# imatge-upc/rsis

Measured on AMD Instinct MI355X. Metric: training images/sec at 256x256, T=10, batch=32 per GPU, higher is better.
Workload: dtype f32

## Files before the change

rsis_amd/csrc/conv_wgrad_tiled.hip:

```cpp
#include "common.h"
#include "launchers.h"
#include "limb_split.h"
#include "wgrad_block_order.h"
#include "wgrad_parts.h"
#include <stdlib.h>
#include <string.h>

typedef __bf16 wg_bf16x8 __attribute__((ext_vector_type(8)));
typedef unsigned wg_u32x4 __attribute__((ext_vector_type(4)));

#define WG_LIMB_PRODUCTS 6
[[maybe_unused]] __device__ constexpr int wg_limb_pa[9] = {2, 1, 0, 1, 0, 0, 2, 1, 2};
[[maybe_unused]] __device__ constexpr int wg_limb_pb[9] = {0, 1, 2, 0, 1, 0, 1, 2, 2};

__device__ __forceinline__ void wg_limb_pack8(const float (&v)[8], wg_bf16x8 (&out)[3]) {
  wg_u32x4 q[3];
#pragma unroll
  for (int m = 0; m < 4; ++m) {
    float lo[3], hi[3];
    rsis_limb_split3(v[2 * m], lo[0], lo[1], lo[2]);
    rsis_limb_split3(v[2 * m + 1], hi[0], hi[1], hi[2]);
    q[0][m] = __builtin_amdgcn_perm(__float_as_uint(v[2 * m + 1]), __float_as_uint(v[2 * m]), 0x07060302u);
    q[1][m] = __builtin_amdgcn_perm(__float_as_uint(hi[1]), __float_as_uint(lo[1]), 0x07060302u);
    q[2][m] = __builtin_amdgcn_perm(__float_as_uint(hi[2]), __float_as_uint(lo[2]), 0x07060302u);
  }
#pragma unroll
  for (int l = 0; l < 3; ++l) out[l] = __builtin_bit_cast(wg_bf16x8, q[l]);
}

struct WgradTiledArgs {
  const float* dy;
  const float* x;
  float* dw;
  int B, Cs, H, W, Cout;
  int ldo, n_off, interleave_hid;
  int n_co_tiles, n_n_tiles, n_sp_tiles, tiles_per_split;
};

template <int BM, int BN, int WGM, int WGN, int KS, int TW, int KSP = 1, int RAG = 0, int LIMB = 0>
__device__ __forceinline__ void wgrad_tiled_body(const WgradTiledArgs& p, const int bx, const int by) {
#if __HIP_DEVICE_COMPILE__
  constexpr int TM = BM / WGM / 32, TN = BN / WGN / 32;
  constexpr int KK = KS * KS, HALO = KS / 2;
  constexpr int TP = KS == 1 ? 32 : 64;
  constexpr int TH = TP / TW;
  constexpr int NG = TP / 4;
  constexpr int GPR = TW / 4;
  constexpr int PW = TW + 2 * HALO, PH = TH + 2 * HALO, IMS = PW * PH;
  constexpr int CI_P = KS == 1 ? BN : (BN + KK - 2) / KK + 1;
  constexpr int AS = BM * TP;
  constexpr int XS = KS == 1 ? BN * TP : (CI_P * IMS + 255) / 256 * 256;
  constexpr int NA = BM * NG / 256;
  constexpr int NB4 = KS == 1 ? BN * NG / 256 : 0;
  constexpr int NB1 = KS == 1 ? 0 : XS / 256;
  static_assert(WGM * WGN * KSP == 4 && (BM * NG) % 256 == 0 && (KS == 3 || (BN * NG) % 256 == 0) && (NG / 2) % KSP == 0 && (NG / 2 / KSP) % 2 == 0, "config");

  __shared__ __attribute__((aligned(16))) float lds[2 * (AS + XS)];
  float* const As0 = lds;
  float* const Xs0 = lds + 2 * AS;

  const int tid = threadIdx.x, lane = tid & 63, l31 = lane & 31, hi = lane >> 5;
  const int wave = __builtin_amdgcn_readfirstlane(tid >> 6);
  const int wk = wave / (WGM * WGN), wm = (wave % (WGM * WGN)) / WGN, wn = wave % WGN;
  const int H = p.H, W = p.W, HW = H * W, Cs = p.Cs, Cout = p.Cout;
  const int co_t = bx % p.n_co_tiles, n_t = bx / p.n_co_tiles;
  const int co0 = co_t * BM, n0 = n_t * BN;
  const int ci0 = n0 / KK;
  const int Nn = Cs * KK;
  const int tiles_x = RAG ? (W + TW - 1) / TW : W / TW, tiles_y = RAG ? (H + TH - 1) / TH : H / TH;
  const int rx = W - (tiles_x - 1) * TW, ry = H - (tiles_y - 1) * TH;
  const int t_begin = by * p.tiles_per_split;
  const int t_end = min(t_begin + p.tiles_per_split, p.n_sp_tiles);
  if (t_begin >= t_end) return;

  unsigned voa[NA];
#pragma unroll
  for (int i = 0; i < NA; ++i) {
    const int idx = tid + i * 256;
    const int row = idx / NG, sl = idx % NG;
    const int G = (sl & ~7) | ((sl & 7) ^ (row & 7));
    const int y = G / GPR, x4 = G % GPR;
    voa[i] = co0 + row < Cout ? ((unsigned)((co0 + row) * HW + y * W + x4 * 4) * 4u) | (RAG == 2 && x4 * 4 >= rx ? 1u : 0u) | (RAG == 2 && y >= ry ? 2u : 0u) : RSIS_OOB;
  }
  unsigned voa1[RAG == 1 ? 4 * NA : 1];
  unsigned vob1r[RAG == 1 && NB4 ? 4 * NB4 : 1];
  if constexpr (RAG == 1) {
#pragma unroll
    for (int k = 0; k < 4 * NA; ++k) {
      const int P = k * 256 + tid, idx = P >> 2, e = P & 3;
      const int row = idx / NG, sl = idx % NG;
      const int G = (sl & ~7) | ((sl & 7) ^ (row & 7));
      const int y = G / GPR, x = (G % GPR) * 4 + e;
      voa1[k] = co0 + row < Cout ? ((unsigned)((co0 + row) * HW + y * W + x) * 4u) | (x >= rx ? 1u : 0u) | (y >= ry ? 2u : 0u) : RSIS_OOB;
    }
    if constexpr (KS == 1) {
#pragma unroll
      for (int k = 0; k < 4 * NB4; ++k) {
        const int P = k * 256 + tid, idx = P >> 2, e = P & 3;
        const int row = idx / NG, sl = idx % NG;
        const int G = (sl & ~7) | ((sl & 7) ^ (row & 7));
        const int y = G / GPR, x = (G % GPR) * 4 + e;
        vob1r[k] = n0 + row < Cs ? ((unsigned)((n0 + row) * HW + y * W + x) * 4u) | (x >= rx ? 1u : 0u) | (y >= ry ? 2u : 0u) : RSIS_OOB;
      }
    }
  }
  unsigned vob4[NB4 ? NB4 : 1];
  unsigned vob1[NB1 ? NB1 : 1];
  unsigned cls1[NB1 ? NB1 : 1];
  if constexpr (KS == 1) {
#pragma unroll
    for (int i = 0; i < NB4; ++i) {
      const int idx = tid + i * 256;
      const int row = idx / NG, sl = idx % NG;
      const int G = (sl & ~7) | ((sl & 7) ^ (row & 7));
      const int y = G / GPR, x4 = G % GPR;
      vob4[i] = n0 + row < Cs ? ((unsigned)((n0 + row) * HW + y * W + x4 * 4) * 4u) | (RAG == 2 && x4 * 4 >= rx ? 1u : 0u) | (RAG == 2 && y >= ry ? 2u : 0u) : RSIS_OOB;
    }
  } else {
#pragma unroll
    for (int i = 0; i < NB1; ++i) {
      const int e = tid + i * 256;
      const int cl = e / IMS, rem = e - cl * IMS;
      const int py = rem / PW, pxx = rem - py * PW;
      const bool ok = cl < CI_P && ci0 + cl < Cs;
      vob1[i] = ok ? (unsigned)(cl * HW + py * W + pxx) * 4u : RSIS_OOB;
      cls1[i] = (py == 0 ? 1u : 0u) | (py - 1 >= ry ? 2u : 0u) | (pxx == 0 ? 4u : 0u) | (pxx - 1 >= rx ? 8u : 0u);
    }
  }

  int sg[NG / 2 / KSP];
  int bo[NG / 2 / KSP];
#pragma unroll
  for (int gg = 0; gg < NG / 2 / KSP; ++gg) {
    const int g = gg * KSP + (KSP == 1 ? 0 : wk);
    sg[gg] = ((2 * g + hi) ^ (l31 & 7)) * 4;
    bo[gg] = KS == 1 ? 0 : (g / (TW / 8)) * PW + (g % (TW / 8)) * 8;
  }
  const int arow = (wm * TM * 32 + l31) * TP;
  int xb[TN];
#pragma unroll
  for (int j = 0; j < TN; ++j) {
    const int nl = wn * TN * 32 + j * 32 + l31;
    if constexpr (KS == 1) {
      xb[j] = nl * TP;
    } else {
      const int n = n0 + nl;
      const int cl = n / KK - ci0, rs = n - (n / KK) * KK;
      xb[j] = cl * IMS + (rs / KS) * PW + (rs % KS) + 4 * hi;
    }
  }

  f32x16 acc[TM][TN];
#pragma unroll
  for (int i = 0; i < TM; ++i)
#pragma unroll
    for (int j = 0; j < TN; ++j)
#pragma unroll
      for (int r = 0; r < 16; ++r) acc[i][j][r] = 0.f;

  int tb = t_begin / (tiles_x * tiles_y);
  int trem = t_begin - tb * (tiles_x * tiles_y);
  int ty = trem / tiles_x, tx = trem - ty * tiles_x;

#define WG_ISSUE(BUF)                                                                                          \
  {                                                                                                            \
    const int y0 = ty * TH, x0 = tx * TW;                                                                      \
    const float* ab = p.dy + ((size_t)tb * Cout * HW + y0 * W + x0);                                           \
    const __amdgpu_buffer_rsrc_t ra_ = __builtin_amdgcn_make_buffer_rsrc((void*)ab, 0, 0x7FFFFFF0, 0x00020000); \
    const unsigned lastm = (tx == tiles_x - 1 ? 1u : 0u) | (ty == tiles_y - 1 ? 2u : 0u);                      \
    if constexpr (RAG == 1) {                                                                                  \
      float* As = As0 + (BUF) * AS + wave * 64;                                                                \
      _Pragma("unroll") for (int k = 0; k < 4 * NA; ++k)                                                       \
        __builtin_amdgcn_raw_ptr_buffer_load_lds(ra_, (lds_vp_t)(As + k * 256), 4, (voa1[k] & lastm) ? RSIS_OOB : (voa1[k] & ~3u), 0, 0, 0); \
    } else {                                                                                                   \
      float* As = As0 + (BUF) * AS + wave * 256;                                                               \
      _Pragma("unroll") for (int i = 0; i < NA; ++i)                                                           \
        __builtin_amdgcn_raw_ptr_buffer_load_lds(ra_, (lds_vp_t)(As + i * 1024), 16,                           \
                                                 RAG == 2 ? ((voa[i] & lastm) ? RSIS_OOB : (voa[i] & ~3u)) : voa[i], 0, 0, 0); \
    }                                                                                                          \
    if constexpr (KS == 1) {                                                                                   \
      const float* bb = p.x + ((size_t)tb * Cs * HW + y0 * W + x0);                                            \
      const __amdgpu_buffer_rsrc_t rb_ = __builtin_amdgcn_make_buffer_rsrc((void*)bb, 0, 0x7FFFFFF0, 0x00020000); \
      if constexpr (RAG == 1) {                                                                                \
        float* Xs = Xs0 + (BUF) * XS + wave * 64;                                                              \
        _Pragma("unroll") for (int k = 0; k < 4 * NB4; ++k)                                                    \
          __builtin_amdgcn_raw_ptr_buffer_load_lds(rb_, (lds_vp_t)(Xs + k * 256), 4, (vob1r[k] & lastm) ? RSIS_OOB : (vob1r[k] & ~3u), 0, 0, 0); \
      } else {                                                                                                 \
        float* Xs = Xs0 + (BUF) * XS + wave * 256;                                                             \
        _Pragma("unroll") for (int i = 0; i < NB4; ++i)                                                        \
          __builtin_amdgcn_raw_ptr_buffer_load_lds(rb_, (lds_vp_t)(Xs + i * 1024), 16,                         \
                                                   RAG == 2 ? ((vob4[i] & lastm) ? RSIS_OOB : (vob4[i] & ~3u)) : vob4[i], 0, 0, 0); \
      }                                                                                                        \
    } else {                                                                                                   \
      const float* bb = p.x + (((size_t)tb * Cs + ci0) * HW + (y0 - 1) * W + (x0 - 1));                        \
      const __amdgpu_buffer_rsrc_t rb_ = __builtin_amdgcn_make_buffer_rsrc((void*)bb, 0, 0x7FFFFFF0, 0x00020000); \
      const unsigned edge = (y0 == 0 ? 1u : 0u) | (ty == tiles_y - 1 ? 2u : 0u) | (x0 == 0 ? 4u : 0u) | (tx == tiles_x - 1 ? 8u : 0u); \
      float* Xs = Xs0 + (BUF) * XS + wave * 64;                                                                \
      _Pragma("unroll") for (int i = 0; i < NB1; ++i) {                                                        \
        const unsigned vo = (cls1[i] & edge) ? RSIS_OOB : vob1[i];                                             \
        __builtin_amdgcn_raw_ptr_buffer_load_lds(rb_, (lds_vp_t)(Xs + i * 256), 4, vo, 0, 0, 0);               \
      }                                                                                                        \
    }                                                                                                          \
    if (++tx == tiles_x) { tx = 0; if (++ty == tiles_y) { ty = 0; ++tb; } }                                    \
  }
#define WG_LAND() __builtin_amdgcn_s_waitcnt(0x0F70);

  WG_ISSUE(0)
  WG_LAND()
  __syncthreads();
  const int ntl = t_end - t_begin;
  for (int t = 0; t < ntl; ++t) {
    const int cur = t & 1;
    if (t + 1 < ntl) WG_ISSUE(cur ^ 1)
    {
      const float* As = As0 + cur * AS + arow;
      const float* Xs = Xs0 + cur * XS;
      if constexpr (LIMB) {
#pragma unroll
        for (int g = 0; g < NG / 2 / KSP; g += 2) {
          wg_bf16x8 al[TM][3], bl[TN][3];
#pragma unroll
          for (int i = 0; i < TM; ++i) {
            const f32x4 a0 = *reinterpret_cast<const f32x4*>(As + i * 32 * TP + sg[g]);
            const f32x4 a1 = *reinterpret_cast<const f32x4*>(As + i * 32 * TP + sg[g + 1]);
            const float v[8] = {a0[0], a0[1], a0[2], a0[3], a1[0], a1[1], a1[2], a1[3]};
            wg_limb_pack8(v, al[i]);
          }
#pragma unroll
          for (int j = 0; j < TN; ++j) {
            float v[8];
            if constexpr (KS == 1) {
              const f32x4 b0 = *reinterpret_cast<const f32x4*>(Xs + xb[j] + sg[g]);
              const f32x4 b1 = *reinterpret_cast<const f32x4*>(Xs + xb[j] + sg[g + 1]);
#pragma unroll
              for (int e = 0; e < 4; ++e) { v[e] = b0[e]; v[4 + e] = b1[e]; }
            } else {
#pragma unroll
              for (int u = 0; u < 2; ++u)
#pragma unroll
                for (int e = 0; e < 4; ++e)
                  v[4 * u + e] = Xs[xb[j] + (KSP == 1 ? ((g + u) / (TW / 8)) * PW + ((g + u) % (TW / 8)) * 8 : bo[g + u]) + e];
            }
            wg_limb_pack8(v, bl[j]);
          }
#pragma unroll
          for (int q = 0; q < WG_LIMB_PRODUCTS; ++q)
#pragma unroll
            for (int i = 0; i < TM; ++i)
#pragma unroll
              for (int j = 0; j < TN; ++j)
                acc[i][j] = __builtin_amdgcn_mfma_f32_32x32x16_bf16(al[i][wg_limb_pa[q]], bl[j][wg_limb_pb[q]], acc[i][j], 0, 0, 0);
        }
      } else
#pragma unroll
      for (int g = 0; g < NG / 2 / KSP; ++g) {
        f32x4 a4[TM];
#pragma unroll
        for (int i = 0; i < TM; ++i) a4[i] = *reinterpret_cast<const f32x4*>(As + i * 32 * TP + sg[g]);
        if constexpr (KS == 1) {
          f32x4 b4[TN];
#pragma unroll
          for (int j = 0; j < TN; ++j) b4[j] = *reinterpret_cast<const f32x4*>(Xs + xb[j] + sg[g]);
#pragma unroll
          for (int e = 0; e < 4; ++e)
#pragma unroll
            for (int i = 0; i < TM; ++i)
#pragma unroll
              for (int j = 0; j < TN; ++j) acc[i][j] = __builtin_amdgcn_mfma_f32_32x32x2f32(a4[i][e], b4[j][e], acc[i][j], 0, 0, 0);
        } else {
#pragma unroll
          for (int e = 0; e < 4; ++e) {
            float b[TN];
#pragma unroll
            for (int j = 0; j < TN; ++j) b[j] = Xs[xb[j] + (KSP == 1 ? (g / (TW / 8)) * PW + (g % (TW / 8)) * 8 : bo[g]) + e];
#pragma unroll
            for (int i = 0; i < TM; ++i)
#pragma unroll
              for (int j = 0; j < TN; ++j) acc[i][j] = __builtin_amdgcn_mfma_f32_32x32x2f32(a4[i][e], b[j], acc[i][j], 0, 0, 0);
          }
        }
      }
    }
    WG_LAND()
    __syncthreads();
  }
#undef WG_ISSUE
#undef WG_LAND

  wg_atomic_tiles<TM, TN>(acc, p.dw, Cout, p.ldo, p.n_off, p.interleave_hid, co0 + wm * TM * 32 + 4 * hi, n0 + wn * TN * 32 + l31, Nn);
#endif
}

#define RSIS_WG_MAXJ 48
struct WgradTiledGroup {
  int n;
  int xcd_order;
  int begin[RSIS_WG_MAXJ + 1];
  WgradTiledArgs job[RSIS_WG_MAXJ];
};
static_assert(sizeof(WgradTiledGroup) <= 4000, "kernel arguments are limited to 4 KB");

template <int BM, int BN, int WGM, int WGN, int KS, int TW, int KSP = 1, int RAG = 0, int LIMB = 0>
__global__ __launch_bounds__(256) void conv_wgrad_tiled_group_kernel(const WgradTiledGroup g) {
  const int b = g.xcd_order ? rsis_xcd_logical_block(blockIdx.x, gridDim.x) : (int)blockIdx.x;
  int lo = 0, hi = g.n - 1;
  while (lo < hi) {
    const int mid = (lo + hi + 1) >> 1;
    if (g.begin[mid] <= b) lo = mid; else hi = mid - 1;
  }
  const WgradTiledArgs& p = g.job[lo];
  const int local = b - g.begin[lo];
  const int ntile = p.n_co_tiles * p.n_n_tiles;
  wgrad_tiled_body<BM, BN, WGM, WGN, KS, TW, KSP, RAG, LIMB>(p, local % ntile, local / ntile);
}

static unsigned wg_limb_mask(int ks, int tw) {
  if (ks == 3) return tw == 16 ? 0x3Fu : (tw == 8 ? 1u << 5 : 0u);
  return (tw == 16 || tw == 8 ? 1u << 2 : 0u) | 1u << 5;
}
static bool wg_use_limbs(int ks, int tw, int code, int rag) {
  static const int mode = [] {
    const char* e = getenv("RSIS_WGRAD_LIMBS");
    if (!e || !e[0]) return 0;
    if (e[0] == '0') return 1;
    return strcmp(e, "all") == 0 ? 2 : 0;
  }();
  if (mode) return mode == 2;
  return rag == 0 && ((wg_limb_mask(ks, tw) >> code) & 1u);
}

static unsigned wg_xcd_mask(int ks, int tw) {
  if (ks == 3) return tw == 16 ? 0x5u : 0u;
  return tw == 32 ? 1u << 5 : 0u;
}
static int wg_xcd_order(int ks, int tw, int code, int rag) {
  static const int mode = [] {
    const char* e = getenv("RSIS_WGRAD_XCD");
    if (!e || !e[0]) return 0;
    if (e[0] == '0') return 1;
    return strcmp(e, "all") == 0 ? 2 : 0;
  }();
  if (mode) return mode == 2;
  return rag == 0 && ((wg_xcd_mask(ks, tw) >> code) & 1u);
}
static constexpr int tiled_code_of(int bm, int bn) { return bm == 32 ? (bn == 64 ? 0 : 1) : (bm == 64 ? (bn == 64 ? 2 : 3) : (bn == 64 ? 4 : 5)); }

static int tiled_tw(int H, int W, int ks) {
  const int tp = ks == 1 ? 32 : 64;
  for (int tw = ks == 1 ? 32 : 16; tw >= 8; tw >>= 1)
    if (W % tw == 0 && H % (tp / tw) == 0) return tw;
  return 0;
}
static int tiled_tw_ragged(int W, int ks) {
  const int wide = ks == 1 ? 32 : 16;
  return W > 16 ? wide : (W > 8 ? 16 : 8);
}

static int tiled_cfg_code_single(const WgradTiledArgs& a, int ks) {
  const int nmod = (a.Cs * ks * ks) % 128;
  const bool narrow = nmod != 0 && nmod <= 64;
  if (ks == 1 && a.Cout > 32) return 2;
  if (a.Cout <= 32) return narrow && !rsis_deterministic() ? 0 : 1;
  if (a.Cout <= 64) return narrow ? 2 : 3;
  return narrow ? 4 : 5;
}

static int wg_job_class(const WgradTiledArgs& a, int ks) {
  if (ks == 1) return a.Cout <= 32 ? -1 : (a.Cout >= 128 && a.Cs >= 128 ? 1 : 0);
  const int nmod = (a.Cs * ks * ks) % 128;
  if (nmod == 0 || nmod > 64) return -1;
  return a.Cout <= 32 ? 0 : (a.Cout <= 64 ? 1 : 2);
}
static int wg_wide_code(int ks, int cls) { return ks == 1 ? 5 : 2 * cls + 1; }
static int wg_group_tile(int ks, int tw, int cls) {
  return ks == 1 && cls == 1 && (tw == 32 || tw == 16) ? 5 : -1;
}
static int tiled_cfg_code(const WgradTiledArgs& a, int ks, int tw, bool grouped) {
  static const int mode = [] {
    const char* e = getenv("RSIS_WGRAD_TILES");
    if (!e || !e[0]) return 0;
    if (strcmp(e, "0") == 0) return 1;
    return strcmp(e, "wide") == 0 ? 2 : 0;
  }();
  const int single = tiled_cfg_code_single(a, ks);
  const int cls = wg_job_class(a, ks);
  if (!grouped || cls < 0 || mode == 1 || rsis_deterministic()) return single;
  const int code = mode == 2 ? wg_wide_code(ks, cls) : wg_group_tile(ks, tw, cls);
  return code < 0 ? single : code;
}

static void tiled_split_plan(WgradTiledArgs* jobs, int n, int ks, bool big_tile, bool alone, int rag) {
  if (alone && rag == 0) {
    WgradTiledArgs& a = jobs[0];
    const int ntile = a.n_co_tiles * a.n_n_tiles;
    const int slots = ks == 1 ? (big_tile ? 256 : 512) : 256 * (big_tile ? 2 : 3);
    int nsplit = ntile >= slots ? 1 : slots / ntile;
    if (nsplit > a.n_sp_tiles / 2) nsplit = a.n_sp_tiles / 2;
    if (nsplit < 1 || rsis_deterministic()) nsplit = 1;
    a.tiles_per_split = rsis_cdiv(a.n_sp_tiles, nsplit);
    return;
  }
  long total_iters = 0;
  for (int j = 0; j < n; ++j) total_iters += (long)jobs[j].n_co_tiles * jobs[j].n_n_tiles * jobs[j].n_sp_tiles;
  static const int env_tb = getenv("RSIS_WG_GROUP_BLOCKS") ? atoi(getenv("RSIS_WG_GROUP_BLOCKS")) : 0;
  const long target_blocks = env_tb > 0 ? env_tb : 2048;
  long L = (total_iters + target_blocks - 1) / target_blocks;
  if (L < 2) L = 2;
  if (rsis_deterministic()) L = 1L << 40;
  for (int j = 0; j < n; ++j) {
    int nsplit = rsis_cdiv(jobs[j].n_sp_tiles, L);
    if (nsplit < 1) nsplit = 1;
    jobs[j].tiles_per_split = rsis_cdiv(jobs[j].n_sp_tiles, nsplit);
  }
}

template <int BM, int BN, int WGM, int WGN, int KS, int TW, int KSP = 1, int RAG = 0, int LIMB = 0>
static int launch_group_cfg(WgradTiledArgs* jobs, int n, bool alone, hipStream_t st) {
  constexpr int TH = (KS == 1 ? 32 : 64) / TW;
  for (int j = 0; j < n; ++j) {
    WgradTiledArgs& a = jobs[j];
    a.n_co_tiles = rsis_cdiv(a.Cout, BM);
    a.n_n_tiles = rsis_cdiv((long)a.Cs * KS * KS, BN);
    a.n_sp_tiles = RAG ? a.B * rsis_cdiv(a.H, TH) * rsis_cdiv(a.W, TW) : a.B * (a.H / TH) * (a.W / TW);
  }
  tiled_split_plan(jobs, n, KS, BM * BN >= 128 * 128, alone, RAG);
  for (int j0 = 0; j0 < n; j0 += RSIS_WG_MAXJ) {
    WgradTiledGroup g;
    g.xcd_order = !alone && wg_xcd_order(KS, TW, tiled_code_of(BM, BN), RAG);
    g.n = n - j0 < RSIS_WG_MAXJ ? n - j0 : RSIS_WG_MAXJ;
    int blocks = 0;
    for (int j = 0; j < g.n; ++j) {
      const WgradTiledArgs& a = jobs[j0 + j];
      g.begin[j] = blocks;
      g.job[j] = a;
      blocks += a.n_co_tiles * a.n_n_tiles * rsis_cdiv(a.n_sp_tiles, a.tiles_per_split);
    }
    g.begin[g.n] = blocks;
    hipLaunchKernelGGL((conv_wgrad_tiled_group_kernel<BM, BN, WGM, WGN, KS, TW, KSP, RAG, LIMB>), dim3(blocks), dim3(256), 0, st, g);
    if (rsis_check_launch() != RSIS_OK) return RSIS_ERR_LAUNCH;
  }
  return RSIS_OK;
}

template <int KS, int TW, int RAG, int LIMB>
static int launch_group_code(int code, WgradTiledArgs* jobs, int n, bool alone, hipStream_t st) {
  switch (code) {
    case 0: return launch_group_cfg<32, 64, 1, 2, KS, TW, 2, RAG, LIMB>(jobs, n, alone, st);
    case 1: return launch_group_cfg<32, 128, 1, 4, KS, TW, 1, RAG, LIMB>(jobs, n, alone, st);
    case 2: return launch_group_cfg<64, 64, 2, 2, KS, TW, 1, RAG, LIMB>(jobs, n, alone, st);
    case 3: return launch_group_cfg<64, 128, 2, 2, KS, TW, 1, RAG, LIMB>(jobs, n, alone, st);
    case 4: return launch_group_cfg<128, 64, 2, 2, KS, TW, 1, RAG, LIMB>(jobs, n, alone, st);
    default: return launch_group_cfg<128, 128, 2, 2, KS, TW, 1, RAG, LIMB>(jobs, n, alone, st);
  }
}

template <int KS, int TW>
static int launch_group_tw(int rag, int code, WgradTiledArgs* jobs, int n, bool alone, hipStream_t st) {
  const bool limb = wg_use_limbs(KS, TW, code, rag);
  switch (rag * 2 + limb) {
    case 0: return launch_group_code<KS, TW, 0, 0>(code, jobs, n, alone, st);
    case 1: return launch_group_code<KS, TW, 0, 1>(code, jobs, n, alone, st);
    case 2: return launch_group_code<KS, TW, 1, 0>(code, jobs, n, alone, st);
    case 3: return launch_group_code<KS, TW, 1, 1>(code, jobs, n, alone, st);
    case 4: return launch_group_code<KS, TW, 2, 0>(code, jobs, n, alone, st);
    default: return launch_group_code<KS, TW, 2, 1>(code, jobs, n, alone, st);
  }
}

static int launch_group(int ks, int tw, int rag, int code, WgradTiledArgs* jobs, int n, bool alone, hipStream_t st) {
  if (ks == 1 && tw == 32) return launch_group_tw<1, 32>(rag, code, jobs, n, alone, st);
  if (ks == 1 && tw == 16) return launch_group_tw<1, 16>(rag, code, jobs, n, alone, st);
  if (ks == 1 && tw == 8) return launch_group_tw<1, 8>(rag, code, jobs, n, alone, st);
  if (ks == 3 && tw == 16) return launch_group_tw<3, 16>(rag, code, jobs, n, alone, st);
  if (ks == 3 && tw == 8) return launch_group_tw<3, 8>(rag, code, jobs, n, alone, st);
  return RSIS_ERR_ARG;
}

static WgradTiledArgs tiled_args(const WgradArgs& w) {
  WgradTiledArgs a = {};
  a.dy = w.dy; a.x = w.x; a.dw = w.dw; a.B = w.B; a.Cs = w.Cs; a.H = w.H; a.W = w.W; a.Cout = w.Cout;
  a.ldo = w.ldo; a.n_off = w.n_off; a.interleave_hid = w.interleave_hid;
  return a;
}

static int tiled_launch_jobs(const WgradArgs* w, int n, int ks, bool alone, hipStream_t st) {
  if (n < 1) return RSIS_OK;
  WgradTiledArgs* all = (WgradTiledArgs*)malloc(sizeof(WgradTiledArgs) * n * 2);
  int* key = (int*)malloc(sizeof(int) * n);
  if (!all || !key) { free(all); free(key); return RSIS_ERR_LAUNCH; }
  WgradTiledArgs* bucket = all + n;
  for (int j = 0; j < n; ++j) {
    WgradTiledArgs& a = all[j] = tiled_args(w[j]);
    const int twa = tiled_tw(a.H, a.W, ks);
    if (twa) key[j] = twa * 8 + tiled_cfg_code(a, ks, twa, !alone);
    else {
      if (ks == 1 && (a.H * a.W) % 4 == 0) { a.W = a.H * a.W; a.H = 1; }
      key[j] = (a.W % 4 == 0 ? 2048 : 1024) + tiled_tw_ragged(a.W, ks) * 8 + tiled_cfg_code_single(a, ks);
    }
  }
  int rc = RSIS_OK;
  for (int j = 0; j < n && rc == RSIS_OK; ++j) {
    if (key[j] < 0) continue;
    const int k = key[j];
    int m = 0;
    for (int i = j; i < n; ++i)
      if (key[i] == k) { bucket[m++] = all[i]; key[i] = -1; }
    rc = launch_group(ks, (k & 1023) / 8, k >> 10, k % 8, bucket, m, alone, st);
  }
  free(all); free(key);
  return rc;
}

int rsis_launch_conv_wgrad_tiled_group(const WgradArgs* w, int n, int ks, hipStream_t st) { return tiled_launch_jobs(w, n, ks, false, st); }
int rsis_launch_conv_wgrad_tiled(const WgradArgs& w, int ks, hipStream_t st) { return tiled_launch_jobs(&w, 1, ks, true, st); }

bool rsis_wgrad_tiled_supported(const WgradArgs& w, int ks) {
  if (!(ks == 1 || ks == 3) || w.stride != 1 || w.pad != ks / 2 || w.H != w.Ho || w.W != w.Wo) return false;
  static const bool ragged_on = !(getenv("RSIS_WGRAD_RAGGED") && getenv("RSIS_WGRAD_RAGGED")[0] == '0');
  if (tiled_tw(w.H, w.W, ks) == 0 && !ragged_on) return false;
  const long img = (long)w.H * w.W * 4;
  return (long)w.Cout * img < (1L << 30) && (long)w.Cs * img < (1L << 30);
}
```

Before: 970.2.

## Extend tiled MFMA weight-gradient kernel to stride-2 3x3 and 7x7 convolutions

Adds a stride-2 variant of the tiled weight-gradient kernel. It stages a full-resolution input patch into LDS with 16-byte buffer loads and reads it with stride-2 offsets. Stride-2 3x3 convolutions and 7x7 convolutions with few input channels now use this path instead of the previous fallback. The limb path accumulates each tile into a separate register partial before adding it to the main accumulator. This costs extra registers but should reduce rounding error.

```diff
diff --git a/rsis_amd/csrc/conv_wgrad_tiled.hip b/rsis_amd/csrc/conv_wgrad_tiled.hip
--- a/rsis_amd/csrc/conv_wgrad_tiled.hip
+++ b/rsis_amd/csrc/conv_wgrad_tiled.hip
@@ -3,6 +3,7 @@
 #include "limb_split.h"
 #include "wgrad_block_order.h"
 #include "wgrad_parts.h"
+#include "wgrad_strided_map.h"
 #include <stdlib.h>
 #include <string.h>
 
@@ -37,7 +38,7 @@
   int n_co_tiles, n_n_tiles, n_sp_tiles, tiles_per_split;
 };
 
-template <int BM, int BN, int WGM, int WGN, int KS, int TW, int KSP = 1, int RAG = 0, int LIMB = 0>
+template <int BM, int BN, int WGM, int WGN, int KS, int TW, int KSP = 1, int RAG = 0, int LIMB = 0, int STR = 1>
 __device__ __forceinline__ void wgrad_tiled_body(const WgradTiledArgs& p, const int bx, const int by) {
 #if __HIP_DEVICE_COMPILE__
   constexpr int TM = BM / WGM / 32, TN = BN / WGN / 32;
@@ -46,14 +47,17 @@
   constexpr int TH = TP / TW;
   constexpr int NG = TP / 4;
   constexpr int GPR = TW / 4;
-  constexpr int PW = TW + 2 * HALO, PH = TH + 2 * HALO, IMS = PW * PH;
+  constexpr int PW = STR == 2 ? wgs2_pitch(KS, TW) : TW + 2 * HALO;
+  constexpr int IMS = STR == 2 ? wgs2_chan(KS, TW, TH) : PW * (TH + 2 * HALO);
   constexpr int CI_P = KS == 1 ? BN : (BN + KK - 2) / KK + 1;
   constexpr int AS = BM * TP;
-  constexpr int XS = KS == 1 ? BN * TP : (CI_P * IMS + 255) / 256 * 256;
+  constexpr int XS = KS == 1 ? BN * TP : (STR == 2 ? wgs2_groups(KS, TW, TH, CI_P) * 4 : (CI_P * IMS + 255) / 256 * 256);
   constexpr int NA = BM * NG / 256;
   constexpr int NB4 = KS == 1 ? BN * NG / 256 : 0;
-  constexpr int NB1 = KS == 1 ? 0 : XS / 256;
-  static_assert(WGM * WGN * KSP == 4 && (BM * NG) % 256 == 0 && (KS == 3 || (BN * NG) % 256 == 0) && (NG / 2) % KSP == 0 && (NG / 2 / KSP) % 2 == 0, "config");
+  constexpr int NB1 = KS == 1 ? 0 : (STR == 2 ? (XS / 4 + 255) / 256 : XS / 256);
+  static_assert(WGM * WGN * KSP == 4 && (BM * NG) % 256 == 0 && (KS != 1 || (BN * NG) % 256 == 0) && (NG / 2) % KSP == 0 && (NG / 2 / KSP) % 2 == 0, "config");
+  static_assert(STR == 1 ? KS == 1 || KS == 3 : STR == 2 && (KS == 3 || KS == 7) && RAG == 0, "stride 2: 3x3 / 7x7 on maps of whole tiles");
+  static_assert(2 * (AS + XS) * 4 <= WG_CU_LDS, "LDS of a CU");
 
   __shared__ __attribute__((aligned(16))) float lds[2 * (AS + XS)];
   float* const As0 = lds;
@@ -63,6 +67,7 @@
   const int wave = __builtin_amdgcn_readfirstlane(tid >> 6);
   const int wk = wave / (WGM * WGN), wm = (wave % (WGM * WGN)) / WGN, wn = wave % WGN;
   const int H = p.H, W = p.W, HW = H * W, Cs = p.Cs, Cout = p.Cout;
+  const int Wx = STR * W, HWx = STR * STR * HW;
   const int co_t = bx % p.n_co_tiles, n_t = bx / p.n_co_tiles;
   const int co0 = co_t * BM, n0 = n_t * BN;
   const int ci0 = n0 / KK;
@@ -120,6 +125,12 @@
 #pragma unroll
     for (int i = 0; i < NB1; ++i) {
       const int e = tid + i * 256;
+      if constexpr (STR == 2) {
+        const WgS2Group s = wgs2_group(KS, TW, TH, CI_P, e);
+        vob1[i] = s.staged && ci0 + s.cl < Cs ? (unsigned)(s.cl * HWx + s.row * Wx + 4 * s.g4) * 4u : RSIS_OOB;
+        cls1[i] = wgs2_class(KS, TW, TH, s.row, s.g4);
+        continue;
+      }
       const int cl = e / IMS, rem = e - cl * IMS;
       const int py = rem / PW, pxx = rem - py * PW;
       const bool ok = cl < CI_P && ci0 + cl < Cs;
@@ -134,7 +145,7 @@
   for (int gg = 0; gg < NG / 2 / KSP; ++gg) {
     const int g = gg * KSP + (KSP == 1 ? 0 : wk);
     sg[gg] = ((2 * g + hi) ^ (l31 & 7)) * 4;
-    bo[gg] = KS == 1 ? 0 : (g / (TW / 8)) * PW + (g % (TW / 8)) * 8;
+    bo[gg] = KS == 1 ? 0 : STR * ((g / (TW / 8)) * PW + (g % (TW / 8)) * 8);
   }
   const int arow = (wm * TM * 32 + l31) * TP;
   int xb[TN];
@@ -146,7 +157,7 @@
     } else {
       const int n = n0 + nl;
       const int cl = n / KK - ci0, rs = n - (n / KK) * KK;
-      xb[j] = cl * IMS + (rs / KS) * PW + (rs % KS) + 4 * hi;
+      xb[j] = (STR == 2 ? wgs2_base(KS, TW, TH, cl, rs / KS, rs % KS) : cl * IMS + (rs / KS) * PW + (rs % KS)) + STR * 4 * hi;
     }
   }
 
@@ -192,13 +203,16 @@
                                                    RAG == 2 ? ((vob4[i] & lastm) ? RSIS_OOB : (vob4[i] & ~3u)) : vob4[i], 0, 0, 0); \
       }                                                                                                        \
     } else {                                                                                                   \
-      const float* bb = p.x + (((size_t)tb * Cs + ci0) * HW + (y0 - 1) * W + (x0 - 1));                        \
+      const float* bb = p.x + (((size_t)tb * Cs + ci0) * HWx + (STR * y0 - HALO) * Wx + (STR * x0 - (STR == 2 ? WGS2_LEFT : HALO))); \
       const __amdgpu_buffer_rsrc_t rb_ = __builtin_amdgcn_make_buffer_rsrc((void*)bb, 0, 0x7FFFFFF0, 0x00020000); \
       const unsigned edge = (y0 == 0 ? 1u : 0u) | (ty == tiles_y - 1 ? 2u : 0u) | (x0 == 0 ? 4u : 0u) | (tx == tiles_x - 1 ? 8u : 0u); \
-      float* Xs = Xs0 + (BUF) * XS + wave * 64;                                                                \
+      float* Xs = Xs0 + (BUF) * XS + wave * (STR == 2 ? 256 : 64);                                             \
       _Pragma("unroll") for (int i = 0; i < NB1; ++i) {                                                        \
         const unsigned vo = (cls1[i] & edge) ? RSIS_OOB : vob1[i];                                             \
-        __builtin_amdgcn_raw_ptr_buffer_load_lds(rb_, (lds_vp_t)(Xs + i * 256), 4, vo, 0, 0, 0);               \
+        if constexpr (STR == 2) {                                                                              \
+          if (i * 256 + wave * 64 < XS / 4)            \
+            __builtin_amdgcn_raw_ptr_buffer_load_lds(rb_, (lds_vp_t)(Xs + i * 1024), 16, vo, 0, 0, 0);         \
+        } else __builtin_amdgcn_raw_ptr_buffer_load_lds(rb_, (lds_vp_t)(Xs + i * 256), 4, vo, 0, 0, 0);        \
       }                                                                                                        \
     }                                                                                                          \
     if (++tx == tiles_x) { tx = 0; if (++ty == tiles_y) { ty = 0; ++tb; } }                                    \
@@ -216,6 +230,16 @@
       const float* As = As0 + cur * AS + arow;
       const float* Xs = Xs0 + cur * XS;
       if constexpr (LIMB) {
+        constexpr bool FLUSH = STR == 2;
+        f32x16 part[TM][TN];
+        if constexpr (FLUSH) {
+#pragma unroll
+          for (int i = 0; i < TM; ++i)
+#pragma unroll
+            for (int j = 0; j < TN; ++j)
+#pragma unroll
+              for (int r = 0; r < 16; ++r) part[i][j][r] = 0.f;
+        }
 #pragma unroll
         for (int g = 0; g < NG / 2 / KSP; g += 2) {
           wg_bf16x8 al[TM][3], bl[TN][3];
@@ -239,7 +263,7 @@
               for (int u = 0; u < 2; ++u)
 #pragma unroll
                 for (int e = 0; e < 4; ++e)
-                  v[4 * u + e] = Xs[xb[j] + (KSP == 1 ? ((g + u) / (TW / 8)) * PW + ((g + u) % (TW / 8)) * 8 : bo[g + u]) + e];
+                  v[4 * u + e] = Xs[xb[j] + (KSP == 1 ? STR * (((g + u) / (TW / 8)) * PW + ((g + u) % (TW / 8)) * 8) : bo[g + u]) + STR * e];
             }
             wg_limb_pack8(v, bl[j]);
           }
@@ -249,7 +273,14 @@
             for (int i = 0; i < TM; ++i)
 #pragma unroll
               for (int j = 0; j < TN; ++j)
-                acc[i][j] = __builtin_amdgcn_mfma_f32_32x32x16_bf16(al[i][wg_limb_pa[q]], bl[j][wg_limb_pb[q]], acc[i][j], 0, 0, 0);
+                if constexpr (FLUSH) part[i][j] = __builtin_amdgcn_mfma_f32_32x32x16_bf16(al[i][wg_limb_pa[q]], bl[j][wg_limb_pb[q]], part[i][j], 0, 0, 0);
+                else acc[i][j] = __builtin_amdgcn_mfma_f32_32x32x16_bf16(al[i][wg_limb_pa[q]], bl[j][wg_limb_pb[q]], acc[i][j], 0, 0, 0);
+        }
+        if constexpr (FLUSH) {
+#pragma unroll
+          for (int i = 0; i < TM; ++i)
+#pragma unroll
+            for (int j = 0; j < TN; ++j) acc[i][j] += part[i][j];
         }
       } else
 #pragma unroll
@@ -272,7 +303,7 @@
           for (int e = 0; e < 4; ++e) {
             float b[TN];
 #pragma unroll
-            for (int j = 0; j < TN; ++j) b[j] = Xs[xb[j] + (KSP == 1 ? (g / (TW / 8)) * PW + (g % (TW / 8)) * 8 : bo[g]) + e];
+            for (int j = 0; j < TN; ++j) b[j] = Xs[xb[j] + (KSP == 1 ? STR * ((g / (TW / 8)) * PW + (g % (TW / 8)) * 8) : bo[g]) + STR * e];
 #pragma unroll
             for (int i = 0; i < TM; ++i)
 #pragma unroll
@@ -300,7 +331,7 @@
 };
 static_assert(sizeof(WgradTiledGroup) <= 4000, "kernel arguments are limited to 4 KB");
 
-template <int BM, int BN, int WGM, int WGN, int KS, int TW, int KSP = 1, int RAG = 0, int LIMB = 0>
+template <int BM, int BN, int WGM, int WGN, int KS, int TW, int KSP = 1, int RAG = 0, int LIMB = 0, int STR = 1>
 __global__ __launch_bounds__(256) void conv_wgrad_tiled_group_kernel(const WgradTiledGroup g) {
   const int b = g.xcd_order ? rsis_xcd_logical_block(blockIdx.x, gridDim.x) : (int)blockIdx.x;
   int lo = 0, hi = g.n - 1;
@@ -311,14 +342,30 @@
   const WgradTiledArgs& p = g.job[lo];
   const int local = b - g.begin[lo];
   const int ntile = p.n_co_tiles * p.n_n_tiles;
-  wgrad_tiled_body<BM, BN, WGM, WGN, KS, TW, KSP, RAG, LIMB>(p, local % ntile, local / ntile);
+  wgrad_tiled_body<BM, BN, WGM, WGN, KS, TW, KSP, RAG, LIMB, STR>(p, local % ntile, local / ntile);
 }
 
 static unsigned wg_limb_mask(int ks, int tw) {
   if (ks == 3) return tw == 16 ? 0x3Fu : (tw == 8 ? 1u << 5 : 0u);
   return (tw == 16 || tw == 8 ? 1u << 2 : 0u) | 1u << 5;
 }
-static bool wg_use_limbs(int ks, int tw, int code, int rag) {
+static int wg_s2_class(int ks) { return ks == 7 ? 1 : 0; }
+static unsigned wg_s2_class_mask() { return 0x3u; }
+static unsigned wg_s2_limb_mask() { return 0x1u; }
+static bool wg_s2_on(int ks) {
+  static const int mode = [] {
+    const char* e = getenv("RSIS_WGRAD_S2");
+    if (!e || !e[0]) return -1;
+    if (strcmp(e, "0") == 0) return 0;
+    if (strcmp(e, "3") == 0) return 1;
+    if (strcmp(e, "7") == 0) return 2;
+    return strcmp(e, "all") == 0 ? 3 : -1;
+  }();
+  return ((mode < 0 ? wg_s2_class_mask() : (unsigned)mode) >> wg_s2_class(ks)) & 1u;
+}
+static int wg_s2_code(int ks) { return ks == 7 ? 2 : 3; }
+
+static bool wg_use_limbs(int ks, int tw, int code, int rag, int str = 1) {
   static const int mode = [] {
     const char* e = getenv("RSIS_WGRAD_LIMBS");
     if (!e || !e[0]) return 0;
@@ -326,6 +373,7 @@
     return strcmp(e, "all") == 0 ? 2 : 0;
   }();
   if (mode) return mode == 2;
+  if (str == 2) return (wg_s2_limb_mask() >> wg_s2_class(ks)) & 1u;
   return rag == 0 && ((wg_limb_mask(ks, tw) >> code) & 1u);
 }
 
@@ -333,7 +381,7 @@
   if (ks == 3) return tw == 16 ? 0x5u : 0u;
   return tw == 32 ? 1u << 5 : 0u;
 }
-static int wg_xcd_order(int ks, int tw, int code, int rag) {
+static int wg_xcd_order(int ks, int tw, int code, int rag, int str = 1) {
   static const int mode = [] {
     const char* e = getenv("RSIS_WGRAD_XCD");
     if (!e || !e[0]) return 0;
@@ -341,6 +389,7 @@
     return strcmp(e, "all") == 0 ? 2 : 0;
   }();
   if (mode) return mode == 2;
+  if (str == 2) return 0;
   return rag == 0 && ((wg_xcd_mask(ks, tw) >> code) & 1u);
 }
 static constexpr int tiled_code_of(int bm, int bn) { return bm == 32 ? (bn == 64 ? 0 : 1) : (bm == 64 ? (bn == 64 ? 2 : 3) : (bn == 64 ? 4 : 5)); }
@@ -414,7 +463,7 @@
   }
 }
 
-template <int BM, int BN, int WGM, int WGN, int KS, int TW, int KSP = 1, int RAG = 0, int LIMB = 0>
+template <int BM, int BN, int WGM, int WGN, int KS, int TW, int KSP = 1, int RAG = 0, int LIMB = 0, int STR = 1>
 static int launch_group_cfg(WgradTiledArgs* jobs, int n, bool alone, hipStream_t st) {
   constexpr int TH = (KS == 1 ? 32 : 64) / TW;
   for (int j = 0; j < n; ++j) {
@@ -426,7 +475,7 @@
   tiled_split_plan(jobs, n, KS, BM * BN >= 128 * 128, alone, RAG);
   for (int j0 = 0; j0 < n; j0 += RSIS_WG_MAXJ) {
     WgradTiledGroup g;
-    g.xcd_order = !alone && wg_xcd_order(KS, TW, tiled_code_of(BM, BN), RAG);
+    g.xcd_order = !alone && wg_xcd_order(KS, TW, tiled_code_of(BM, BN), RAG, STR);
     g.n = n - j0 < RSIS_WG_MAXJ ? n - j0 : RSIS_WG_MAXJ;
     int blocks = 0;
     for (int j = 0; j < g.n; ++j) {
@@ -436,7 +485,7 @@
       blocks += a.n_co_tiles * a.n_n_tiles * rsis_cdiv(a.n_sp_tiles, a.tiles_per_split);
     }
     g.begin[g.n] = blocks;
-    hipLaunchKernelGGL((conv_wgrad_tiled_group_kernel<BM, BN, WGM, WGN, KS, TW, KSP, RAG, LIMB>), dim3(blocks), dim3(256), 0, st, g);
+    hipLaunchKernelGGL((conv_wgrad_tiled_group_kernel<BM, BN, WGM, WGN, KS, TW, KSP, RAG, LIMB, STR>), dim3(blocks), dim3(256), 0, st, g);
     if (rsis_check_launch() != RSIS_OK) return RSIS_ERR_LAUNCH;
   }
   return RSIS_OK;
@@ -467,7 +516,26 @@
   }
 }
 
-static int launch_group(int ks, int tw, int rag, int code, WgradTiledArgs* jobs, int n, bool alone, hipStream_t st) {
+template <int KS, int TW>
+static int launch_group_s2(int code, WgradTiledArgs* jobs, int n, bool alone, hipStream_t st) {
+  const bool limb = wg_use_limbs(KS, TW, code, 0, 2);
+  if constexpr (KS == 7) {
+    if (code != 2) return RSIS_ERR_ARG;
+    return limb ? launch_group_cfg<64, 64, 2, 2, KS, TW, 1, 0, 1, 2>(jobs, n, alone, st) : launch_group_cfg<64, 64, 2, 2, KS, TW, 1, 0, 0, 2>(jobs, n, alone, st);
+  } else {
+    if (code != 3) return RSIS_ERR_ARG;
+    return limb ? launch_group_cfg<64, 128, 2, 2, KS, TW, 1, 0, 1, 2>(jobs, n, alone, st) : launch_group_cfg<64, 128, 2, 2, KS, TW, 1, 0, 0, 2>(jobs, n, alone, st);
+  }
+}
+
+static int launch_group(int ks, int str, int tw, int rag, int code, WgradTiledArgs* jobs, int n, bool alone, hipStream_t st) {
+  if (str == 2) {
+    if (ks == 3 && tw == 16) return launch_group_s2<3, 16>(code, jobs, n, alone, st);
+    if (ks == 3 && tw == 8) return launch_group_s2<3, 8>(code, jobs, n, alone, st);
+    if (ks == 7 && tw == 16) return launch_group_s2<7, 16>(code, jobs, n, alone, st);
+    if (ks == 7 && tw == 8) return launch_group_s2<7, 8>(code, jobs, n, alone, st);
+    return RSIS_ERR_ARG;
+  }
   if (ks == 1 && tw == 32) return launch_group_tw<1, 32>(rag, code, jobs, n, alone, st);
   if (ks == 1 && tw == 16) return launch_group_tw<1, 16>(rag, code, jobs, n, alone, st);
   if (ks == 1 && tw == 8) return launch_group_tw<1, 8>(rag, code, jobs, n, alone, st);
@@ -491,6 +559,11 @@
   WgradTiledArgs* bucket = all + n;
   for (int j = 0; j < n; ++j) {
     WgradTiledArgs& a = all[j] = tiled_args(w[j]);
+    if (w[j].stride == 2) {
+      a.H = w[j].Ho; a.W = w[j].Wo;
+      key[j] = 4096 + tiled_tw(a.H, a.W, ks) * 8 + wg_s2_code(ks);
+      continue;
+    }
     const int twa = tiled_tw(a.H, a.W, ks);
     if (twa) key[j] = twa * 8 + tiled_cfg_code(a, ks, twa, !alone);
     else {
@@ -505,7 +578,7 @@
     int m = 0;
     for (int i = j; i < n; ++i)
       if (key[i] == k) { bucket[m++] = all[i]; key[i] = -1; }
-    rc = launch_group(ks, (k & 1023) / 8, k >> 10, k % 8, bucket, m, alone, st);
+    rc = launch_group(ks, k >> 12 ? 2 : 1, (k & 1023) / 8, (k >> 10) & 3, k % 8, bucket, m, alone, st);
   }
   free(all); free(key);
   return rc;
@@ -515,6 +588,13 @@
 int rsis_launch_conv_wgrad_tiled(const WgradArgs& w, int ks, hipStream_t st) { return tiled_launch_jobs(&w, 1, ks, true, st); }
 
 bool rsis_wgrad_tiled_supported(const WgradArgs& w, int ks) {
+  if (w.stride == 2) {
+    if (!((ks == 3 || (ks == 7 && w.Cs <= 4)) && w.pad == ks / 2 && wg_s2_on(ks))) return false;
+    if (w.H != 2 * w.Ho || w.W != 2 * w.Wo || tiled_tw(w.Ho, w.Wo, ks) == 0) return false;
+    if ((size_t)w.x & 15) return false;
+    const long img = (long)w.H * w.W * 4;
+    return (long)w.Cout * img < (1L << 30) && (long)w.Cs * img < (1L << 30);
+  }
   if (!(ks == 1 || ks == 3) || w.stride != 1 || w.pad != ks / 2 || w.H != w.Ho || w.W != w.Wo) return false;
   static const bool ragged_on = !(getenv("RSIS_WGRAD_RAGGED") && getenv("RSIS_WGRAD_RAGGED")[0] == '0');
   if (tiled_tw(w.H, w.W, ks) == 0 && !ragged_on) return false;
diff --git a/rsis_amd/csrc/wgrad_strided_map.h b/rsis_amd/csrc/wgrad_strided_map.h
--- /dev/null
+++ b/rsis_amd/csrc/wgrad_strided_map.h
@@ -0,0 +1,35 @@
+#pragma once
+
+#if defined(__HIPCC__) || defined(__CUDACC__)
+#define RSIS_S2MAP_HD __host__ __device__
+#else
+#define RSIS_S2MAP_HD
+#endif
+
+RSIS_S2MAP_HD constexpr int wgs2_tap_p(int ks, int r) { return (r - ks / 2) & 1; }
+RSIS_S2MAP_HD constexpr int wgs2_tap_a(int ks, int r) { return (r - ks / 2 - wgs2_tap_p(ks, r)) / 2; }
+RSIS_S2MAP_HD constexpr int wgs2_extent(int ks, int t, int p) { return t + (ks / 2 - p) / 2 + (ks / 2 + p) / 2; }
+RSIS_S2MAP_HD constexpr int wgs2_span(int ks, int t) { return wgs2_extent(ks, t, 0) + wgs2_extent(ks, t, 1); }
+
+constexpr int WGS2_LEFT = 4;
+RSIS_S2MAP_HD constexpr int wgs2_pitch(int ks, int tw) { return (WGS2_LEFT - ks / 2 + wgs2_span(ks, tw) + 3) / 4 * 4; }
+RSIS_S2MAP_HD constexpr int wgs2_chan(int ks, int tw, int th) { return wgs2_span(ks, th) * wgs2_pitch(ks, tw) + (ks == 3 ? 4 : 0); }
+RSIS_S2MAP_HD constexpr int wgs2_groups(int ks, int tw, int th, int nch) { return (nch * wgs2_chan(ks, tw, th) / 4 + 63) / 64 * 64; }
+RSIS_S2MAP_HD constexpr int wgs2_base(int ks, int tw, int th, int cl, int r, int s) {
+  return cl * wgs2_chan(ks, tw, th) + r * wgs2_pitch(ks, tw) + s + WGS2_LEFT - ks / 2;
+}
+
+struct WgS2Group { int staged, cl, row, g4; };
+RSIS_S2MAP_HD constexpr WgS2Group wgs2_group(int ks, int tw, int th, int nch, int G) {
+  const int chan4 = wgs2_chan(ks, tw, th) / 4, pitch4 = wgs2_pitch(ks, tw) / 4;
+  const int cl = G / chan4, rem = G - cl * chan4;
+  const int row = rem / pitch4, g4 = rem - row * pitch4;
+  if (cl >= nch || row >= wgs2_span(ks, th)) return WgS2Group{0, 0, 0, 0};
+  return WgS2Group{1, cl, row, g4};
+}
+RSIS_S2MAP_HD constexpr unsigned wgs2_class(int ks, int tw, int th, int row, int g4) {
+  return (row < ks / 2 ? 1u : 0u) | (row >= 2 * th + ks / 2 ? 2u : 0u) | (g4 == 0 ? 4u : 0u) | (4 * g4 - WGS2_LEFT >= 2 * tw ? 8u : 0u);
+}
+RSIS_S2MAP_HD constexpr unsigned wgs2_edge(int ty, int tiles_y, int tx, int tiles_x) {
+  return (ty == 0 ? 1u : 0u) | (ty == tiles_y - 1 ? 2u : 0u) | (tx == 0 ? 4u : 0u) | (tx == tiles_x - 1 ? 8u : 0u);
+}
```

Result: no change. 974.5 (median of 6 runs) (+0.5%).
